# keonlee9420/Comprehensive-Transformer-TTS

Measured on AMD Instinct MI355X. Metric: mel-frames/sec (train step) LJSpeech batch=16, 1/2/4/8 MI355X, higher is better.
Workload: dtype f32; 1 GPU; LJSpeech transformer_fs2 batch=16/GPU seq<=128->mel<=1024x80; full train step fwd+loss+bwd+clip+Adam, dropout on; workload_detail=supervised durations (BASELINE configs[1]), global_batch=16, valid_frames_per_gpu=11992, padded_frames_per_gpu=16384, launch_mode=hipgraph(fwd+bwd | clip+adam), parallelism=dp1

## Files before the change

comprehensive-transformer-tts_amd/_lib.py:

```python
import ctypes as C
import os

_HERE = os.path.dirname(os.path.abspath(__file__))
LIB_PATH = os.environ.get("CTTS_LIB") or os.path.join(_HERE, "csrc", "libctts_hip.so")

_c_f32p = C.c_void_p
_i32, _i64, _f32, _u32, _vp = C.c_int32, C.c_int64, C.c_float, C.c_uint32, C.c_void_p


class GemmDesc(C.Structure):
    _fields_ = [
        ("A", _vp), ("B", _vp), ("C", _vp),
        ("M", _i32), ("N", _i32), ("K", _i32),
        ("lda", _i64), ("ldb", _i64), ("ldc", _i64),
        ("a_kc", _i32), ("b_kc", _i32),
        ("nb0", _i32), ("nb1", _i32),
        ("sA0", _i64), ("sA1", _i64), ("sB0", _i64), ("sB1", _i64), ("sC0", _i64), ("sC1", _i64),
        ("lens", _vp),
        ("lim_m", _i32), ("lim_n", _i32), ("lim_k", _i32),
        ("conv_T", _i32), ("conv_pad", _i32), ("conv_cin", _i32), ("conv_on_b", _i32),
        ("split_k", _i32),
        ("alpha", _f32),
        ("bias", _vp),
        ("Z", _vp), ("ldz", _i64),
# ... 83 lines not shown
    "ctts_gemm_takes_weight_stationary": [C.POINTER(GemmDesc)],
    "ctts_gemm_takes_bf16_split": [C.POINTER(GemmDesc)],
    "ctts_gemm_takes_planes": [C.POINTER(GemmDesc)],
    "ctts_split_planes": [C.POINTER(SplitTask), C.c_int, _vp],
    "ctts_rowdot_heads": [_vp, _vp, _vp, C.c_int, C.c_int, C.c_int, C.c_int, _vp],
    "ctts_mel_prepare": [_vp, C.c_int, C.c_int, _vp, _vp],
    "ctts_mel_spectrogram": [_vp, _vp, _vp, _vp, _vp, _vp, _vp, _i64, C.c_int, C.c_int, C.c_int, C.c_int, C.c_int, _f32, C.c_int, _vp, _vp],
    "ctts_mha_fwd": [_vp, _vp, _vp, _vp, C.c_int, C.c_int, C.c_int, C.c_int, _f32, _vp],
    "ctts_mha_bwd": [_vp, _vp, _vp, _vp, _vp, _vp, _vp, _vp, _vp, C.c_int, C.c_int, C.c_int, C.c_int, _f32, C.c_int, _vp, _vp],
    "ctts_relmha_fwd": [_vp, _vp, _vp, _vp, _vp, _vp, C.c_int, C.c_int, C.c_int, C.c_int, _f32, _f32, _vp, _u32, _vp],
    "ctts_relmha_bwd": [_vp, _vp, _vp, _vp, _vp, _vp, _vp, _vp, _vp, _vp, _vp, _vp, _vp, C.c_int, C.c_int, C.c_int, C.c_int,
                        _f32, _f32, _vp, _u32, _vp],
    "ctts_weighted_colsum": [_vp, _vp, _vp, _i64, C.c_int, _f32, C.c_int, _vp, _vp, _vp],
    "ctts_epilogue_bwd": [_vp, _vp, _vp, _vp, _vp, _vp, _i64, C.c_int, C.c_int, _f32, _vp, _u32, _f32, C.c_int, _vp, _vp, _vp],
    "ctts_row_tile_map": [_vp, C.c_int, C.c_int, C.c_int, _vp, _vp],
    "ctts_conv_weight_repack": [_vp, _vp, C.c_int, C.c_int, C.c_int, C.c_int, _vp],
    "ctts_lr_index": [_vp, C.c_int, C.c_int, _vp, C.c_int, C.c_int, C.c_int, _vp, _vp, _vp, _vp],
    "ctts_lr_gather_fwd": [_vp, _vp, _vp, C.c_int, C.c_int, C.c_int, C.c_int, _vp],
    "ctts_lr_gather_bwd": [_vp, _vp, _vp, C.c_int, C.c_int, C.c_int, C.c_int, _vp],
    "ctts_embedding_fwd": [_vp, _vp, _vp, _i64, C.c_int, C.c_int, _vp],
    "ctts_embedding_bwd": [_vp, _vp, _vp, _i64, C.c_int, C.c_int, C.c_int, C.c_int, _vp, _vp],
    "ctts_positions": [_vp, C.c_int, _i64, C.c_int, C.c_int, _vp, _vp],
    "ctts_cwt_pitch": [_vp, _i64, C.c_int, _vp, _vp, _f32, _vp, C.c_int, _f32, _f32, _f32, C.c_int, _vp, _vp, _vp, C.c_int, C.c_int, C.c_int, _vp],
    "ctts_layernorm_fwd": [_vp, _vp, _vp, _vp, _vp, _vp, C.c_int, C.c_int, _f32, _f32, _vp, _u32, _vp, _vp, _vp],
    "ctts_layernorm_bwd": [_vp, _vp, _vp, _vp, _vp, _vp, _vp, _vp, C.c_int, C.c_int, _f32, _vp, _u32, _vp, C.c_int, _vp, _vp, _vp, _vp],
    "ctts_colstats": [_vp, _vp, C.c_int, C.c_int, _vp, _vp],
    "ctts_bn_finalize": [_vp, C.c_int, C.c_int, _f32, _f32, _vp, _vp, _vp, _vp, _vp, _vp],
    "ctts_bn_apply": [_vp, _vp, _vp, _vp, _vp, _vp, C.c_int, C.c_int, C.c_int, _f32, _vp, _u32, _vp, _vp],
    "ctts_bn_bwd_reduce": [_vp, _vp, _vp, _vp, _vp, _vp, _vp, C.c_int, C.c_int, C.c_int, _f32, _vp, _u32, _vp, _vp],
    "ctts_bn_bwd_apply": [_vp, _vp, _vp, _vp, _vp, _vp, _vp, _vp, _vp, _vp, C.c_int, C.c_int, C.c_int, _f32, _vp,
# ... 76 lines not shown
    "ctts_stoi": [_vp, _vp, _vp, _vp, _vp, _vp, _vp, C.c_int, C.c_int, _vp, _vp],
    "ctts_si_sdr": [_vp, _vp, _vp, _vp, C.c_int, C.c_int, _vp, _vp],
    "ctts_mr_stft": [_vp, _vp, _vp, _vp, _vp, _vp, C.c_int, C.c_int, C.c_int, C.c_int, C.c_int, _vp, _vp],
    "ctts_comm_unique_id": [_vp],
    "ctts_comm_create": [C.POINTER(_vp), _i32, _i32, _vp],
    "ctts_comm_destroy": [_vp],
    "ctts_allreduce_mean": [_vp, _i64, _vp, _vp],
}
COMM_ID_BYTES = 128
EXPORTED_SYMBOLS = sorted(list(_SIGNATURES) + ["ctts_last_error", "ctts_version", "ctts_mha_supported", "ctts_relmha_workspace_floats",
                                               "ctts_mel_spectrogram_workspace_bytes", "ctts_gemm_workspace_bytes", "ctts_workspace_bytes",
                                               "ctts_workspace_error_word", "ctts_fastformer_workspace_floats",
                                               "ctts_griffinlim_workspace_bytes", "ctts_griffinlim_state_floats",
                                               "ctts_pitch_track_workspace_bytes", "ctts_trim_silence_workspace_bytes",
                                               "ctts_dtw_workspace_bytes", "ctts_loudness_workspace_bytes", "ctts_stoi_workspace_bytes",
                                               "ctts_si_sdr_workspace_bytes", "ctts_mr_stft_workspace_bytes"])
ADAM_STATE_FLOATS = 3 + 2048
ABI_VERSION = 2

_lib = None


class CttsError(RuntimeError):
    pass


def load():
    global _lib
    if _lib is not None:
        return _lib
    if not os.path.exists(LIB_PATH):
# ... 31 lines not shown
    lib.ctts_griffinlim_state_floats.argtypes = [C.c_int, C.c_int]
    lib.ctts_pitch_track_workspace_bytes.restype = C.c_size_t
    lib.ctts_pitch_track_workspace_bytes.argtypes = []
    lib.ctts_trim_silence_workspace_bytes.restype = C.c_size_t
    lib.ctts_trim_silence_workspace_bytes.argtypes = [C.c_int, C.c_int, C.c_int]
    lib.ctts_dtw_workspace_bytes.restype = C.c_size_t
    lib.ctts_dtw_workspace_bytes.argtypes = [C.c_int, C.c_int, C.c_int]
    lib.ctts_loudness_workspace_bytes.restype = C.c_size_t
    lib.ctts_loudness_workspace_bytes.argtypes = [C.c_int, C.c_int]
    lib.ctts_stoi_workspace_bytes.restype = C.c_size_t
    lib.ctts_stoi_workspace_bytes.argtypes = [C.c_int, C.c_int]
    lib.ctts_si_sdr_workspace_bytes.restype = C.c_size_t
    lib.ctts_si_sdr_workspace_bytes.argtypes = [C.c_int, C.c_int]
    lib.ctts_mr_stft_workspace_bytes.restype = C.c_size_t
    lib.ctts_mr_stft_workspace_bytes.argtypes = [C.c_int, C.c_int, C.c_int, C.c_int]
    lib.ctts_relmha_workspace_floats.restype = C.c_size_t
    lib.ctts_relmha_workspace_floats.argtypes = [C.c_int, C.c_int, C.c_int]
    _lib = lib
    return lib


def check(status, what):
    if status != 0:
        msg = load().ctts_last_error().decode(errors="replace")
        raise CttsError(f"{what} failed with status {status}: {msg}")
```

comprehensive-transformer-tts_amd/csrc/gemm.hip:

```cpp
#include "ctts_common.h"
#include "gemm_common.h"
#include <stdlib.h>
#include <type_traits>

namespace {

#ifndef CTTS_BK
#define CTTS_BK 32
#endif
#ifndef CTTS_GEMM_WAVES
#define CTTS_GEMM_WAVES 2
#endif
constexpr int BK = CTTS_BK;
constexpr int KC_LD = BK + 4;
constexpr int KCH = BK / 4;
static_assert(BK == 32 || BK == 64, "BK must be 32 or 64");


__device__ __forceinline__ bool rows_in_padding(const int32_t* row_lens, int row_T, int row_halo, int first, int last) {
  const int b0 = first / row_T;
  return b0 == last / row_T && (first - b0 * row_T) >= row_lens[b0] + row_halo;
}

__device__ __forceinline__ void batch_limits(const ctts_gemm_desc& d, int z0, bool apply, int& Mv, int& Nv, int& Kv) {
  Mv = d.M; Nv = d.N; Kv = d.K;
  if (apply && d.lens) {
    const int L = d.lens[z0];
    if (d.lim_m) Mv = min(Mv, L);
    if (d.lim_n) Nv = min(Nv, L);
    if (d.lim_k) Kv = min(Kv, L);
  }
}

__device__ __forceinline__ bool split_k_range(const ctts_gemm_desc& d, int Kv, int granule, int split, int& k_begin, int& k_end) {
  k_begin = 0; k_end = Kv;
  if (d.split_k > 1) {
    const GemmSplitRange s = gemm_split_range(Kv, d.split_k, granule, split);
    k_begin = s.k_begin; k_end = s.k_end;
    if (k_begin >= k_end) return false;
  }
  return true;
}

__device__ __forceinline__ void xcd_tile_order(int nwg, int tiles_n, bool scramble, int& wg, int& tm) {
  const int q8 = nwg >> 3, r8 = nwg & 7, xcd = blockIdx.x & 7, slot = blockIdx.x >> 3;
  wg = (xcd < r8 ? xcd * (q8 + 1) : r8 * (q8 + 1) + (xcd - r8) * q8) + slot;
// ... 363 lines not shown
  }
}

template <int BM, int BN, bool A_KC, bool B_KC, bool CONV, Fetch FETCH>
__global__ __launch_bounds__(256, CTTS_GEMM_WAVES) void gemm_tile_kernel(const ctts_gemm_desc d) {
  using FT = FetchTraits<FETCH>;
  constexpr int WAVES_N = BN >= 64 ? 2 : 1, WAVES_M = 4 / WAVES_N;
  constexpr int WM = BM / WAVES_M, WN = BN / WAVES_N, MT = WM / 32, NT = WN / 32;
  constexpr int A_LD = A_KC ? KC_LD : BM + 4;
  constexpr int B_LD = B_KC ? KC_LD : BN + 4;
  constexpr int A_SZ = A_KC ? BM * KC_LD : BK * (BM + 4);
  constexpr int B_SZ = B_KC ? BN * KC_LD : BK * (BN + 4);
  __shared__ __attribute__((aligned(16))) float smem[A_SZ + B_SZ];
  float* sA = smem;
  float* sB = smem + A_SZ;
  const int z = blockIdx.z;
  const int split = blockIdx.y;
  const int z0 = z / d.nb1, z1 = z - z0 * d.nb1;
  const bool limited = FT::kLensLimits && (FT::kLensGiven || d.lens);
  int Mv, Nv, Kv;
  batch_limits(d, z0, limited, Mv, Nv, Kv);
  const int tiles_n = (d.N + BN - 1) / BN;
  int wg, tm;
  bool scheduled_active = false;
  if (FT::kTileOrders && BM == 64 && A_KC && d.tile_map && !natural_order(d)) {
    wg = blockIdx.x;
    int r = wg / tiles_n;
    if (d.tile_group_n > 0) {
      const int g = d.tile_group_n, ngroups = tiles_n / g, mways = 8 / ngroups;
      const int x = blockIdx.x & 7, i = blockIdx.x >> 3;
      r = (i / g) * mways + x / ngroups;
      wg = r * tiles_n + (x % ngroups) * g + i % g;
    }
    tm = d.tile_map[1 + r];
    scheduled_active = FT::kTrustSchedule && r < d.tile_map[0];
  } else if (FT::kNaturalOrder || (FT::kTileOrders && natural_order(d))) {
    wg = blockIdx.x;
    tm = wg / tiles_n;
  } else {
    xcd_tile_order(gridDim.x, tiles_n, true, wg, tm);
  }
  const int row0 = tm * BM, col0 = (wg % tiles_n) * BN;
  float* Cb = d.C + z0 * d.sC0 + z1 * d.sC1;
  const bool zero_outside = limited && d.split_overwrite && d.split_k <= 1;
  if (row0 >= Mv || col0 >= Nv) {
    if (zero_outside && row0 < d.M && col0 < d.N) zero_outside_limits(d, Cb, row0, col0, BM, BN, Mv, Nv, true);
    return;
  }
  if (zero_outside && (row0 + BM > Mv || col0 + BN > Nv)) zero_outside_limits(d, Cb, row0, col0, BM, BN, Mv, Nv, false);
  float* Cs = Cb;
  if (d.split_k > 1) Cs += (long)split * d.M * d.ldc;
  if (A_KC && d.row_lens && !scheduled_active &&
      padded_tile_zeroed(d, FT::kPadFillOwnSplit ? Cs : Cb, row0, col0, BM, min(BN, Nv - col0), Mv)) return;
  int k_begin, k_end;
  if (!split_k_range(d, Kv, BK, split, k_begin, k_end)) return;

// ... 460 lines not shown
    const unsigned long long m = __ballot(a);
    if (a) map[1 + n_act + __popcll(m & ((1ULL << lane) - 1ULL))] = tm;
    n_act += __popcll(m);
  }
  int n_in = 0;
  for (int base = 0; base < tiles; base += 64) {
    const int tm = base + lane;
    const bool a = tm < tiles && inactive(tm);
    const unsigned long long m = __ballot(a);
    if (a) map[1 + n_act + n_in + __popcll(m & ((1ULL << lane) - 1ULL))] = tm;
    n_in += __popcll(m);
  }
  if (lane == 0) map[0] = n_act;
}

__global__ __launch_bounds__(256) void splitk_reduce_kernel(const ctts_gemm_desc d, int BM, int kround) {
  const int z = blockIdx.z, z0 = z / d.nb1, z1 = z - z0 * d.nb1;
  int Mv, Nv, Kv;
  batch_limits(d, z0, true, Mv, Nv, Kv);
  const bool ow = d.split_overwrite != 0;
  const int nact = Kv > 0 ? gemm_split_range(Kv, d.split_k, kround, 0).nonempty : 0;
  if (nact == 0 && !ow) return;
  const long ldp = gemm_partial_ld(d.N);
  const int n4 = (int)(ldp >> 2);
  const long e = (long)blockIdx.x * 256 + threadIdx.x;
  const int m = (int)(e / n4), n = (int)(e - (long)m * n4) * 4;
  if (m >= d.M || n >= d.N) return;
  bool live = m < Mv && n < Nv && nact > 0;
  if (live && d.a_kc && d.row_lens) {
    const int row0 = m / BM * BM;
// ... 30 lines not shown
int splitk_reduce(const ctts_gemm_desc& d, int BM, int kround, hipStream_t st) {
  const long e = (long)d.M * (gemm_partial_ld(d.N) / 4);
  hipLaunchKernelGGL(splitk_reduce_kernel, dim3((unsigned)((e + 255) / 256), 1, d.nb0 * d.nb1), dim3(256), 0, st, d, BM, kround);
  CTTS_CHECK_LAUNCH("ctts_gemm(split-K reduce)");
  return 0;
}
}

extern "C" int ctts_row_tile_map(const int32_t* row_lens, int row_T, int row_halo, int M, int32_t* tile_map, void* stream) {
  CTTS_REQUIRE(row_lens && tile_map && row_T > 0 && M >= 0, "ctts_row_tile_map: bad arguments");
  hipLaunchKernelGGL(row_tile_map_kernel, dim3(1), dim3(64), 0, (hipStream_t)stream, row_lens, row_T, row_halo, M, tile_map);
  CTTS_CHECK_LAUNCH("ctts_row_tile_map");
  return 0;
}

static bool x6_plan(const ctts_gemm_desc& d) {
  const int on = d.bf16_split;
  static const long min_tiles = ctts_env_int("CTTS_X6_MIN_TILES", 384);
  if (on < 1 || !d.a_kc || !d.b_kc || d.nb0 * d.nb1 != 1 || d.split_k > 1 || d.E || d.lens || d.conv_on_b) return false;
  if (d.K < 256 || d.K % BK || d.N % 128 || d.M < 1024) return false;
  if (d.conv_T > 0 && d.conv_cin % 4) return false;
  if (on != 2 && on != 4 && (long)((d.M + 127) / 128) * (d.N / 128) < min_tiles) return false;
  return vec_ok(d) && buf_ok(d);
}

static bool x6tn_plan(const ctts_gemm_desc& d) {
  static const int tn = ctts_env_int("CTTS_X6_TN", 1);
  static const long min_wg = ctts_env_int("CTTS_X6_TN_MIN_WG", 384);
  if (d.bf16_split < 1 || !tn || d.a_kc || d.b_kc || d.nb0 * d.nb1 != 1 || d.E || d.lens || d.epi_bwd) return false;
  if (d.M % 128 || d.N % 128 || d.K % BK || d.K < 2048) return false;
// ... 6 lines not shown
  const dim3 grid((d.M / 128) * (d.N / 128), d.split_k > 1 ? d.split_k : 1, 1);
  if (d.conv_T > 0) hipLaunchKernelGGL(gemm_x6tn_kernel<true>, grid, dim3(256), 0, st, d);
  else hipLaunchKernelGGL(gemm_x6tn_kernel<false>, grid, dim3(256), 0, st, d);
  CTTS_CHECK_LAUNCH("ctts_gemm(x6tn)");
  return 0;
}

static int x6_launch(const ctts_gemm_desc& d, hipStream_t st) {
  const int tiles = ((d.M + 127) / 128) * (d.N / 128);
  if (d.conv_T > 0) hipLaunchKernelGGL(gemm_x6_kernel<true>, dim3(tiles), dim3(256), 0, st, d);
  else hipLaunchKernelGGL(gemm_x6_kernel<false>, dim3(tiles), dim3(256), 0, st, d);
  CTTS_CHECK_LAUNCH("ctts_gemm(x6)");
  return 0;
}

struct GemmRoute {
  ctts_gemm_route_info info;
  bool split_fits;
  int tile_group_n;
  bool natural_order;
  union { PlArgs pl; PlwArgs plw; WsArgs ws; SkArgs sk; };
  GemmGrid grid;
};

static void tile_plan(const ctts_gemm_desc& d, bool x6tn, GemmRoute& r) {
  const long tiles128 = (long)((d.M + 127) / 128) * ((d.N + 127) / 128) * (d.split_k > 1 ? d.split_k : 1) * d.nb0 * d.nb1;
  static const int force_tile = ctts_env_int("CTTS_FORCE_TILE", 0);
  static const bool natural = getenv("CTTS_NATURAL_ORDER") != nullptr;
  static const int tile_group = ctts_env_int("CTTS_TILE_GROUP", -1);
  if (tile_group != 0 && d.tile_map && d.tile_map != reinterpret_cast<const int32_t*>(1)) {
    const int tn = (d.N + 63) / 64, tmn = (d.M + 63) / 64;
    const int g = tile_group > 0 ? tile_group : ((tn >= 8 && tn % 4 == 0) ? tn / 4 : 0);
    if (g > 0 && tn % g == 0) {
      const int ng = tn / g;
      if ((ng == 1 || ng == 2 || ng == 4 || ng == 8) && tmn % (8 / ng) == 0 && ((long)tmn * tn) % 8 == 0) r.tile_group_n = g;
    }
  }
  static const bool tn_natural = getenv("CTTS_TN_NATURAL") != nullptr;
  r.natural_order = (natural || (tn_natural && !d.a_kc && !d.b_kc)) && !d.tile_map;
  const bool aligned = vec_ok(d);
#ifdef CTTS_NO_BUF
  const bool buf_unaligned = false;
#else
  const bool buf_unaligned = !aligned && chunks_ok(d) && d.conv_T <= 0 && !(d.lens && (d.lim_m || d.lim_n || d.lim_k));
#endif
  r.info.tile_m = r.info.tile_n = 64;
  if (x6tn) { r.info.kind = CTTS_GEMM_X6TN; r.info.tile_m = r.info.tile_n = 128; }
  else if (!aligned && !(buf_unaligned && buf_ok(d))) r.info.kind = CTTS_GEMM_SCALAR64;
#ifndef CTTS_NO_BUF
  else if (buf_ok(d)) {
    static const int k2 = ctts_env_int("CTTS_K2_TILE", 640);
    static const int k2_mink = ctts_env_int("CTTS_K2_MIN_K", 256);
    static const int k2_tn = ctts_env_int("CTTS_K2_TN", 1);
    static const bool narrow = ctts_env_int("CTTS_NARROW_TILE", 1) != 0;
    if (force_tile == 128) { r.info.kind = CTTS_GEMM_BUF128; r.info.tile_m = r.info.tile_n = 128; }
    else if (k2 && (d.a_kc || (k2_tn && !d.b_kc)) && d.nb0 * d.nb1 == 1 && !d.lens && d.N >= 64 && d.M >= 256 && d.K >= k2_mink &&
             (long)((d.M + 63) / 64) * ((d.N + 63) / 64) * (d.split_k > 1 ? d.split_k : 1) <= k2) { r.info.kind = CTTS_GEMM_BUF_K2; r.info.tile_m = 32; }
    else if (narrow && d.N <= 32 && d.M >= 256 && d.conv_T <= 0 && !d.tile_map && !r.natural_order && !d.row_lens) { r.info.kind = CTTS_GEMM_BUF_NARROW; r.info.tile_m = 128; r.info.tile_n = 32; }
    else r.info.kind = CTTS_GEMM_BUF64;
  }
#endif
  else if (tiles128 >= 256 && d.N > 64 && (d.a_kc || d.b_kc)) { r.info.kind = CTTS_GEMM_VEC128; r.info.tile_m = r.info.tile_n = 128; }
  else r.info.kind = CTTS_GEMM_VEC64;
  r.info.k_granule = r.info.kind == CTTS_GEMM_BUF_K2 ? 2 * BK : BK;
}

static void gemm_route(const ctts_gemm_desc& d, GemmRoute& r, bool unbounded_room = false) {
  r.info = ctts_gemm_route_info{CTTS_GEMM_NONE, 128, 128, 1, 32};
  r.split_fits = true;
  r.tile_group_n = 0;
  r.natural_order = false;
  bool x6tn = false;
  if (ctts_gemm_pl_plan(d, r.pl, r.grid)) r.info.kind = CTTS_GEMM_PLANES;
// ... 15 lines not shown
static int gemm_validate(const ctts_gemm_desc* dp, ctts_gemm_desc& d) {
  CTTS_REQUIRE(dp != nullptr, "ctts_gemm: null descriptor");
  d = gemm_normalized(*dp);
  CTTS_REQUIRE(d.A && d.B && d.C, "ctts_gemm: null operand pointer");
  CTTS_REQUIRE(d.M >= 0 && d.N >= 0 && d.K >= 0, "ctts_gemm: negative dimension");
  if (d.M == 0 || d.N == 0) return 1;
  if (d.conv_T > 0) {
    CTTS_REQUIRE(d.conv_cin > 0 && (d.conv_cin % 4) == 0, "ctts_gemm: conv view needs cin %% 4 == 0 (got %d)", d.conv_cin);
    CTTS_REQUIRE(d.conv_on_b ? (!d.a_kc && !d.b_kc) : (d.a_kc != 0), "ctts_gemm: conv view on an unsupported operand layout");
  }
  CTTS_REQUIRE(d.p_drop >= 0.f && d.p_drop < 1.f, "ctts_gemm: p_drop out of range");
  CTTS_REQUIRE(!d.epi_bwd || (d.split_k <= 1 && !d.bias && !d.R && !d.rowscale && !d.E && (!d.act || d.Z)),
               "ctts_gemm: epi_bwd excludes bias, residual, rowscale, E and split-K, and needs Z when an activation is given");
  CTTS_REQUIRE(!d.E || (d.rowsub && d.split_k <= 1 && !d.bias && !d.act && d.p_drop == 0.f && !d.R && !d.rowscale && !d.Z),
               "ctts_gemm: the E/rowsub epilogue excludes bias, activation, dropout, residual, rowscale and split-K");
  return 0;
}

static int gemm_plan(const ctts_gemm_desc* dp, ctts_gemm_desc& d, GemmRoute& r) {
  const int rc = gemm_validate(dp, d);
  if (rc != 0) return rc;
  gemm_route(d, r);
  if (r.info.kind < CTTS_GEMM_X6TN || d.split_k <= 1) return 0;
  CTTS_REQUIRE(d.split_out || (d.sk_ws && d.sk_ws_bytes >= (int64_t)CTTS_WS_BYTES),
               "ctts_gemm: split_k > 1 needs the workspace (ctts_workspace_bytes() bytes, zero-filled once) in sk_ws - partial sums "
               "are added in a fixed order through it, the library has no floating-point atomics");
  CTTS_REQUIRE(r.split_fits, "ctts_gemm: split-K output [%d, %d] x %d batches does not fit the %s", d.M, d.N, d.nb0 * d.nb1,
               d.split_out ? "caller's split_out buffer" : "workspace");
  return 0;
}

extern "C" int ctts_gemm(const ctts_gemm_desc* dp, void* stream) {
  ctts_gemm_desc d;
  GemmRoute r;
  int rc = gemm_plan(dp, d, r);
  if (rc != 0) return rc < 0 ? rc : 0;
  hipStream_t st = reinterpret_cast<hipStream_t>(stream);
// ... 75 lines not shown
```

comprehensive-transformer-tts_amd/kernels.py:

```python
import collections
import ctypes as C

import torch

from . import _lib
from ._lib import GemmDesc

ACT_NONE, ACT_RELU, ACT_GELU, ACT_TANH, ACT_SWISH = 0, 1, 2, 3, 4


def _stream():
    return C.c_void_p(torch.cuda.current_stream().cuda_stream)


def _p(t, offset=0):
    if t is None:
        return None
    if not t.is_cuda:
        raise _lib.CttsError("ctts kernels need device (HIP) tensors; got a CPU tensor - no CPU fallback exists")
    return t.data_ptr() + offset * t.element_size()


def _f32c(t, name):
    if t.dtype != torch.float32 or not t.is_contiguous():
# ... 204 lines not shown
        d.conv_T, d.conv_pad, d.conv_cin = int(conv[0]), int(conv[1]), int(conv[2])
        d.conv_on_b = int(conv_on_b)
    d.split_k = int(split_k)
    d.alpha = float(alpha)
    d.bias = _p(bias)
    d.Z, d.ldz = _p(Z), int(ldz)
    d.act = int(act)
    d.p_drop = float(p_drop)
    d.seed = _p(seed)
    d.drop_offset = int(drop_offset)
    d.R, d.ldr = _p(R), int(ldr)
    d.rowscale = _p(rowscale)
    if row_lens is not None:
        d.row_lens, d.row_T, d.row_halo = _p(row_lens), int(row_T), int(row_halo)
        d.tile_map = _p(tile_map)
    d.E, d.rowsub = _p(E), _p(rowsub)
    d.epi_bwd = int(bool(epi_bwd))
    d.split_overwrite = int(bool(split_overwrite))
    if int(split_k) > 1 or a_planes is not None or ((SK_ENABLED if use_sk is None else use_sk) and nb0 * nb1 == 1 and M * N * K >= (1 << 24)):
        ws = gemm_workspace(A.device)
        d.sk_ws, d.sk_ws_bytes = ws.data_ptr(), ws.numel()
    return d


def gemm(A, B, Cout, M, N, K, lda, ldb, ldc, a_kc=True, b_kc=True, defer=False, **kw):
    d = _gemm_desc(A, B, Cout, M, N, K, lda, ldb, ldc, a_kc, b_kc, **kw)
    lib = _lib.load()
    if defer and _SINK is not None and d.split_k > 1 and d.nb0 * d.nb1 == 1 and ldc == N and N % 4 == 0:
        cnt, stride = C.c_int32(0), C.c_int64(0)
        if lib.ctts_gemm_split_plan(C.byref(d), C.byref(cnt), C.byref(stride)) == 1:
# ... 152 lines not shown
    return pl[:, :, q, :].reshape(pl.shape[0], -1)


def gemm_takes_weight_stationary(A, B, Cout, M, N, K, lda, ldb, ldc, a_kc=True, b_kc=True, **kw):
    return _gemm_takes("weight_stationary", (A, B, Cout, M, N, K, lda, ldb, ldc, a_kc, b_kc), kw)


def gemm_ws_enable(on):
    return bool(_lib.load().ctts_gemm_ws_enable(1 if on else 0))


def row_tile_map(row_lens, row_T, row_halo, M):
    tm = torch.empty(1 + (M + 63) // 64, dtype=torch.int32, device=row_lens.device)
    lib = _lib.load()
    _lib.check(lib.ctts_row_tile_map(_p(row_lens), int(row_T), int(row_halo), int(M), _p(tm), _stream()), "ctts_row_tile_map")
    return tm


def conv_dgrad_weights(weights):
    if not weights:
        return []
    outs = [torch.empty(cin, k * cout, dtype=torch.float32, device=w.device) for w, cout, cin, k in weights]
    arr = (_lib.RepackTask * len(weights))()
    for t, (w, cout, cin, k), o in zip(arr, weights, outs):
        t.src, t.dst, t.cout, t.cin, t.k = _p(_f32c(w, "conv weight (GEMM-major)")), _p(o), int(cout), int(cin), int(k)
    _lib.check(_lib.load().ctts_conv_dgrad_weights(arr, len(arr), _stream()), "ctts_conv_dgrad_weights")
    return outs


def conv_weight_repack(src, dst, cout, cin, k, mode):
# ... 1482 lines not shown
```

comprehensive-transformer-tts_amd/model.py:

```python
import json
import math
import os

import torch
import torch.nn as nn
import torch.nn.functional as F

from . import kernels as K
from . import ops
from .configs import N_SYMBOLS

F0_BIN = 256
F0_MEL_MIN = 1127 * math.log(1 + 50.0 / 700)
F0_MEL_MAX = 1127 * math.log(1 + 1100.0 / 700)


class _Linear(nn.Module):
    def __init__(self, cin, cout, bias=True):
        super().__init__()
        self.weight = nn.Parameter(torch.empty(cout, cin))
        self.bias = nn.Parameter(torch.empty(cout)) if bias else None


class _Conv(nn.Module):
# ... 124 lines not shown
        p = self.dropout if self.training else 0.0
        drop = self.drop_ctx if p > 0 else None
        nonpad, lens = mask_aux(pad_mask)
        if self.use_pos_embed:
            x = self.embed_positions.add_to(x.contiguous(), x, C, self.pos_embed_alpha, nonpad, p, drop)
        else:
            x = ops.rowscale_dropout(x, nonpad, 0.0, None)
        alpha = self.ksize ** -0.5
        pr = ops.PadRows(lens, T)
        for li, layer in enumerate(self.layers):
            op = layer.op
            if self._cut_prefix is not None:
                x = ops.stage_cut(x, f"{self._cut_prefix}.{li}")
            h, xr = ops.layer_norm_res(x, op.layer_norm1.weight, op.layer_norm1.bias, 1e-12)
            qkv = ops.linear(h, op.self_attn.in_proj_weight, pad_rows=pr)
            a = ops.self_attention(qkv, lens, self.num_heads)
            x = ops.linear(a, op.self_attn.out_proj.weight, None, residual=xr, rowscale=nonpad, p_drop=p, drop=drop, pad_rows=pr)
            h, xr = ops.layer_norm_res(x, op.layer_norm2.weight, op.layer_norm2.bias, 1e-12,
                                       planes_for=(op.ffn.conv1.weight.shape[0], self.ksize))
            link = ops.EpiLink()
            g = ops.conv1d(h, op.ffn.conv1.weight, op.ffn.conv1.bias, act=self.ffn_act, alpha=alpha, p_drop=p, drop=drop,
                           pad_rows=pr, link=link, link_role=1, padding=self.ffn_padding)
            x = ops.linear(g, op.ffn.ffn_2.weight, op.ffn.ffn_2.bias, residual=xr, rowscale=nonpad, p_drop=p, drop=drop,
                           pad_rows=pr, link=link, link_role=2)
        return ops.layer_norm(x, self.layer_norm.weight, self.layer_norm.bias, 1e-5, rowscale=nonpad)

    def forward(self, x, padding_mask=None):
        if padding_mask is None:
            padding_mask = x.abs().sum(-1).eq(0)
        return self.run(x, padding_mask), padding_mask

# ... 621 lines not shown
```

comprehensive-transformer-tts_amd/ops.py:

```python
import contextlib
import math
import os as _os

import torch

from . import kernels as K
from .kernels import ACT_NONE, ACT_RELU, ACT_GELU, ACT_TANH, ACT_SWISH


_FUSE_GRAD_ACCUM = False


def set_grad_accumulation_fusion(flag):
    global _FUSE_GRAD_ACCUM
    _FUSE_GRAD_ACCUM = bool(flag)


def grad_accumulation_fusion():
    return _FUSE_GRAD_ACCUM


def _grad_of(p):
    if not _FUSE_GRAD_ACCUM or p is None or not p.requires_grad:
        return None
# ... 447 lines not shown
    for (kind, w), pl in zip(slots, K.split_planes(mats)):
        _PLANES[kind][w.data_ptr()] = (pl, _wstamp(w))


def clear_dgrad_weights():
    _DGRAD_W.clear()
    _PLANES["fwd"].clear()
    _PLANES["dgrad"].clear()


class PadRows:

    def __init__(self, lens, T):
        self.lens, self.T = lens, int(T)
        self._maps = {}

    def tile_map(self, halo, M):
        key = (int(halo), int(M))
        if key not in self._maps:
            self._maps[key] = K.row_tile_map(self.lens, self.T, halo, M)
        return self._maps[key]


def _pad_rows(pad_rows):
    if pad_rows is None or isinstance(pad_rows, PadRows):
        return pad_rows
    return PadRows(pad_rows[0], pad_rows[1])


def linear(x, w, b=None, act=ACT_NONE, alpha=1.0, residual=None, rowscale=None, p_drop=0.0, drop=None, pad_rows=None, link=None,
           link_role=0):
    p_drop, seed, off = _drop_args(p_drop, drop)
    return _LinearConv.apply(x, w, b, residual, rowscale, act, alpha, p_drop, seed, off, 0, 0, _pad_rows(pad_rows), link, link_role)


def conv1d(x, w, b=None, act=ACT_NONE, alpha=1.0, residual=None, rowscale=None, p_drop=0.0, drop=None, pad_rows=None, link=None,
# ... 107 lines not shown
    Cc = x.shape[-1]
    return bool(x.is_cuda and K.PRODUCER_PLANES and K.plane_shape_ok(x.numel() // Cc, int(cout), int(ksize) * Cc, Cc))


def layer_norm_res(x, gamma, beta, eps, planes_for=None):
    want = planes_for is not None and consumer_takes_planes(x, *planes_for)
    return _LayerNormRes.apply(x, gamma, beta, eps, want)


def layer_norm(x, gamma, beta, eps, rowscale=None, p_drop=0.0, drop=None):
    p_drop, seed, off = _drop_args(p_drop, drop)
    return _LayerNorm.apply(x, gamma, beta, eps, rowscale, p_drop, seed, off)


_ATTN_SPLIT_K = int(_os.environ.get("CTTS_ATTN_SPLIT_K", "1"))


def _attn_split_k(nbatch, T, dh):
    tiles = -(-T // 64) * -(-dh // 64) * nbatch
    return _ATTN_SPLIT_K if (_ATTN_SPLIT_K > 1 and tiles < 1536 and T >= 512) else 1


_FUSED_ATTN = {"1": True, "0": False}.get(_os.environ.get("CTTS_FUSED_ATTN", "auto"), None)
_ATTN_Q_SPLIT = int(_os.environ.get("CTTS_ATTN_Q_SPLIT", "0"))


def set_fused_attention(flag):
    global _FUSED_ATTN
    _FUSED_ATTN = flag if flag is None else bool(flag)

# ... 15 lines not shown
        H = ctx.n_heads
        B, T, C3 = qkv.shape
        dh = C3 // 3 // H
        qs = _ATTN_Q_SPLIT if _ATTN_Q_SPLIT > 0 else (2 if (B * H * ((T + 31) // 32) <= 2048 and T >= 256) else 1)
        return K.mha_bwd(qkv, lens, out, dO.contiguous(), lse, H, dh ** -0.5, qs), None, None


def _heads(x, H, parts=1):
    B, T, Cc = x.shape
    return x.view(B, T, parts, H, Cc // (parts * H)).permute(2, 0, 3, 1, 4).unbind(0)


class _SelfAttention(torch.autograd.Function):

    @staticmethod
    def forward(ctx, qkv, lens, n_heads):
        qkv = qkv.contiguous()
        B, T, C3 = qkv.shape
        C = C3 // 3
        dh = C // n_heads
        q, k, v = _heads(qkv, n_heads, 3)
        S = torch.empty(B, n_heads, T, T, dtype=torch.float32, device=qkv.device)
        K.bgemm(q, k.transpose(-1, -2), S, lens=lens, lim=(1, 1, 0), alpha=dh ** -0.5)
        K.softmax_fwd(S, lens, B, n_heads, T)
        sk = _attn_split_k(B * n_heads, T, dh)
        out = torch.empty(B, T, C, dtype=torch.float32, device=qkv.device)
        K.bgemm(S, v, _heads(out, n_heads)[0], lens=lens, lim=(1, 0, 1), split_k=sk, split_overwrite=True)
        ctx.save_for_backward(qkv, S, lens, out)
        ctx.n_heads = n_heads
        return out

    @staticmethod
    def backward(ctx, dO):
        qkv, P, lens, O = ctx.saved_tensors
        H = ctx.n_heads
        dO = dO.contiguous()
        B, T, C3 = qkv.shape
        dh = C3 // 3 // H
        scale = dh ** -0.5
        sk = _attn_split_k(B * H, T, dh)
        dqkv = torch.empty_like(qkv)
        (q, k, v), (dq, dk, dv), (dOh,) = _heads(qkv, H, 3), _heads(dqkv, H, 3), _heads(dO, H)
        K.bgemm(P.transpose(-1, -2), dOh, dv, lens=lens, lim=(1, 0, 1), split_k=sk, split_overwrite=True)
        Dv = K.rowdot_heads(dO, O, H)
        dP = torch.empty_like(P)
        K.bgemm(dOh, v.transpose(-1, -2), dP, lens=lens, lim=(1, 1, 0), E=P, rowsub=Dv)
        K.bgemm(dP, k, dq, lens=lens, lim=(1, 0, 1), alpha=scale, split_k=sk, split_overwrite=True)
        K.bgemm(dP.transpose(-1, -2), q, dk, lens=lens, lim=(1, 0, 1), alpha=scale, split_k=sk, split_overwrite=True)
        return dqkv, None, None


def self_attention(qkv, lens_i32, n_heads):
    want = _FUSED_ATTN if _FUSED_ATTN is not None else not (torch.is_grad_enabled() and qkv.requires_grad)
    if want and K.mha_supported(qkv.shape[-1] // 3, n_heads):
        return _FusedSelfAttention.apply(qkv, lens_i32, n_heads)
    return _SelfAttention.apply(qkv, lens_i32, n_heads)


class _LRGather(torch.autograd.Function):
    @staticmethod
    def forward(ctx, x, mel2ph, cum):
        x = x.contiguous()
        ctx.save_for_backward(cum)
        ctx.Ts = x.shape[1]
        return K.lr_gather_fwd(x, mel2ph)

    @staticmethod
    def backward(ctx, dy):
        (cum,) = ctx.saved_tensors
        return K.lr_gather_bwd(dy.contiguous(), cum, ctx.Ts), None, None

# ... 819 lines not shown
```

include/ctts.h:

```cpp
#ifndef CTTS_H
#define CTTS_H
#include <stddef.h>
#include <stdint.h>

#ifdef __cplusplus
extern "C" {
#endif

const char* ctts_last_error(void);
int ctts_version(void);

typedef struct ctts_gemm_desc {
  const float* A; const float* B; float* C;
  int32_t M, N, K;
  int64_t lda, ldb, ldc;
  int32_t a_kc, b_kc;
  int32_t nb0, nb1;
  int64_t sA0, sA1, sB0, sB1, sC0, sC1;
  const int32_t* lens;
  int32_t lim_m, lim_n, lim_k;
  int32_t conv_T, conv_pad, conv_cin, conv_on_b;
  int32_t split_k;
  float alpha;
  const float* bias;
// ... 49 lines not shown
int ctts_gemm_takes_planes(const ctts_gemm_desc* d);
typedef struct ctts_split_task { const float* src; uint16_t* dst; int64_t rows, cols, ld; } ctts_split_task;
int ctts_split_planes(const ctts_split_task* tasks, int ntasks, void* stream);

int ctts_rowdot_heads(const float* a, const float* b, float* out, int B, int T, int H, int dh, void* stream);

int ctts_weighted_colsum(const float* x, const float* w, float* out, int64_t rows, int C, float scale, int accumulate, void* ws, float* parts,
                         void* stream);

int ctts_epilogue_bwd(const float* dy, const float* rowscale, const float* z, float* dz, float* gm, float* dbias, int64_t rows, int C,
                      int act, float p_drop, const uint64_t* seed, uint32_t drop_offset, float bias_scale, int accumulate_bias,
                      void* ws, float* parts, void* stream);

int ctts_row_tile_map(const int32_t* row_lens, int row_T, int row_halo, int M, int32_t* tile_map, void* stream);

int ctts_conv_weight_repack(const float* src, float* dst, int cout, int cin, int k, int mode, void* stream);

int ctts_lr_index(const void* dur, int dur_is_float, int round_mode, const uint8_t* pad, int B, int Ts, int Tm,
                  int32_t* mel2ph, int64_t* mel_len, int32_t* cum, void* stream);
int ctts_lr_gather_fwd(const float* x, const int32_t* mel2ph, float* out, int B, int Ts, int Tm, int C, void* stream);
int ctts_lr_gather_bwd(const float* dy, const int32_t* cum, float* dx, int B, int Ts, int Tm, int C, void* stream);

int ctts_cwt_pitch(const float* spec, int64_t ld_spec, int nscale, const float* f0_mean, const float* f0_std, float std_scale,
                   const float* uv, int uv_chan, float eps, float mel_min, float mel_max, int f0_bin, float* f0, float* f0_denorm,
                   int64_t* ids, int B, int T, int width, void* stream);

int ctts_positions(const void* src, int src_is_float, int64_t stride, int B, int T, int32_t* pos, void* stream);

int ctts_layernorm_fwd(const float* x, const float* gamma, const float* beta, float* y, float* mean, float* rstd,
                       int rows, int C, float eps, float p_drop, const uint64_t* seed, uint32_t drop_offset,
// ... 246 lines not shown
```

Before: 681,300 mel-frames/s.

## Schedule batched attention GEMM tiles by per-batch work with a device-built plan

Adds a device-side batch tile plan for variable-length batched GEMMs in the unfused self-attention path. It lists the active tiles of every batch, orders them by K-work in a snake pattern across CU bins, and lets the 64x64 buffer kernel launch only the active tiles, returning early for the rest. The goal is to cut idle workgroups and load imbalance from padded sequences in the attention bgemms. In exchange it adds an extra plan kernel per shape, a per-workgroup indirection through the plan, and new routing constraints (no split-K, buf64 kernel only).

```diff
diff --git a/comprehensive-transformer-tts_amd/_lib.py b/comprehensive-transformer-tts_amd/_lib.py
--- a/comprehensive-transformer-tts_amd/_lib.py
+++ b/comprehensive-transformer-tts_amd/_lib.py
@@ -121,6 +121,7 @@
     "ctts_weighted_colsum": [_vp, _vp, _vp, _i64, C.c_int, _f32, C.c_int, _vp, _vp, _vp],
     "ctts_epilogue_bwd": [_vp, _vp, _vp, _vp, _vp, _vp, _i64, C.c_int, C.c_int, _f32, _vp, _u32, _f32, C.c_int, _vp, _vp, _vp],
     "ctts_row_tile_map": [_vp, C.c_int, C.c_int, C.c_int, _vp, _vp],
+    "ctts_batch_tile_map": [_vp] + [C.c_int] * 9 + [_vp, C.c_size_t, _vp],
     "ctts_conv_weight_repack": [_vp, _vp, C.c_int, C.c_int, C.c_int, C.c_int, _vp],
     "ctts_lr_index": [_vp, C.c_int, C.c_int, _vp, C.c_int, C.c_int, C.c_int, _vp, _vp, _vp, _vp],
     "ctts_lr_gather_fwd": [_vp, _vp, _vp, C.c_int, C.c_int, C.c_int, C.c_int, _vp],
@@ -227,7 +228,8 @@
                                                "ctts_griffinlim_workspace_bytes", "ctts_griffinlim_state_floats",
                                                "ctts_pitch_track_workspace_bytes", "ctts_trim_silence_workspace_bytes",
                                                "ctts_dtw_workspace_bytes", "ctts_loudness_workspace_bytes", "ctts_stoi_workspace_bytes",
-                                               "ctts_si_sdr_workspace_bytes", "ctts_mr_stft_workspace_bytes"])
+                                               "ctts_si_sdr_workspace_bytes", "ctts_mr_stft_workspace_bytes",
+                                               "ctts_batch_tile_map_ints"])
 ADAM_STATE_FLOATS = 3 + 2048
 ABI_VERSION = 2
 
@@ -289,6 +291,8 @@
     lib.ctts_si_sdr_workspace_bytes.argtypes = [C.c_int, C.c_int]
     lib.ctts_mr_stft_workspace_bytes.restype = C.c_size_t
     lib.ctts_mr_stft_workspace_bytes.argtypes = [C.c_int, C.c_int, C.c_int, C.c_int]
+    lib.ctts_batch_tile_map_ints.restype = C.c_size_t
+    lib.ctts_batch_tile_map_ints.argtypes = [C.c_int, C.c_int, C.c_int, C.c_int]
     lib.ctts_relmha_workspace_floats.restype = C.c_size_t
     lib.ctts_relmha_workspace_floats.argtypes = [C.c_int, C.c_int, C.c_int]
     _lib = lib
diff --git a/comprehensive-transformer-tts_amd/csrc/batch_plan.h b/comprehensive-transformer-tts_amd/csrc/batch_plan.h
--- /dev/null
+++ b/comprehensive-transformer-tts_amd/csrc/batch_plan.h
@@ -0,0 +1,76 @@
+#pragma once
+#include <stdint.h>
+#ifdef __HIPCC__
+#define BP_HD __host__ __device__ __forceinline__
+#else
+#define BP_HD inline
+#endif
+
+struct BatchPlanGeom {
+  int M, N, K;
+  int BM, BN, BK;
+  int nbatch, nb1;
+  int lim_m, lim_n, lim_k;
+  int write_all;
+  int nbins;
+};
+
+constexpr int BATCH_PLAN_HDR = 4;
+
+BP_HD int batch_plan_tiles_m(const BatchPlanGeom& g) { return (g.M + g.BM - 1) / g.BM; }
+BP_HD int batch_plan_tiles_n(const BatchPlanGeom& g) { return (g.N + g.BN - 1) / g.BN; }
+BP_HD long batch_plan_items(const BatchPlanGeom& g) { return (long)g.nbatch * batch_plan_tiles_m(g) * batch_plan_tiles_n(g); }
+
+BP_HD bool batch_plan_fits(const BatchPlanGeom& g) {
+  const long tiles = (long)batch_plan_tiles_m(g) * batch_plan_tiles_n(g);
+  return g.nbatch >= 1 && g.nb1 >= 1 && g.nbins >= 1 && tiles >= 1 && tiles <= 65536 && g.nbatch <= 32767 &&
+         tiles * g.nbatch * g.nbatch <= (1L << 26);
+}
+BP_HD int32_t batch_plan_pack(int z, int tile) { return (int32_t)((z << 16) | tile); }
+BP_HD void batch_plan_unpack(int32_t e, int& z, int& tile) { z = (int)((uint32_t)e >> 16); tile = e & 0xFFFF; }
+
+BP_HD int32_t batch_plan_key(const BatchPlanGeom& g) {
+  return (int32_t)((g.lim_m & 1) | (g.lim_n & 1) << 1 | (g.lim_k & 1) << 2 | (g.write_all & 1) << 3 | (batch_plan_tiles_n(g) & 0xFFF) << 4 |
+                   (g.BM & 0xFF) << 16 | (g.BN & 0xFF) << 24);
+}
+
+struct BatchPlanBatch {
+  int work;
+  int act_m, act_n;
+};
+
+BP_HD BatchPlanBatch batch_plan_batch(const BatchPlanGeom& g, int L) {
+  const int Mv = g.lim_m && L < g.M ? L : g.M, Nv = g.lim_n && L < g.N ? L : g.N, Kv = g.lim_k && L < g.K ? L : g.K;
+  BatchPlanBatch b;
+  b.work = Kv > 0 ? (Kv + g.BK - 1) / g.BK : 0;
+  b.act_m = Mv > 0 ? (Mv + g.BM - 1) / g.BM : 0;
+  b.act_n = Nv > 0 ? (Nv + g.BN - 1) / g.BN : 0;
+  if (b.act_m == 0 || b.act_n == 0) b.act_m = b.act_n = 0;
+  return b;
+}
+
+BP_HD int batch_plan_snake(int p, int n_active, int nbins) {
+  const int layer = p / nbins, r = p - layer * nbins;
+  const int width = n_active - layer * nbins < nbins ? n_active - layer * nbins : nbins;
+  return layer * nbins + ((layer & 1) ? width - 1 - r : r);
+}
+
+BP_HD int batch_plan_slot(const BatchPlanGeom& g, const int32_t* lens, int z, int tile, int& n_active) {
+  const int tiles_n = batch_plan_tiles_n(g), tiles = batch_plan_tiles_m(g) * tiles_n;
+  const BatchPlanBatch me = batch_plan_batch(g, lens[z / g.nb1]);
+  int act_before = 0, rest_before = 0, total = 0;
+  for (int y = 0; y < g.nbatch; ++y) {
+    const BatchPlanBatch o = batch_plan_batch(g, lens[y / g.nb1]);
+    const int a = o.act_m * o.act_n;
+    total += a;
+    if (o.work > me.work || (o.work == me.work && y < z)) act_before += a;
+    if (y < z) rest_before += tiles - a;
+  }
+  n_active = total;
+  const int tm = tile / tiles_n, tn = tile - tm * tiles_n;
+  const int act_in = (tm < me.act_m ? tm : me.act_m) * me.act_n + (tm < me.act_m ? (tn < me.act_n ? tn : me.act_n) : 0);
+  if (tm < me.act_m && tn < me.act_n) return batch_plan_snake(act_before + act_in, total, g.nbins);
+  return total + rest_before + (tile - act_in);
+}
+
+BP_HD int batch_plan_listed(const BatchPlanGeom& g, int n_active) { return g.write_all ? (int)batch_plan_items(g) : n_active; }
diff --git a/comprehensive-transformer-tts_amd/csrc/gemm.hip b/comprehensive-transformer-tts_amd/csrc/gemm.hip
--- a/comprehensive-transformer-tts_amd/csrc/gemm.hip
+++ b/comprehensive-transformer-tts_amd/csrc/gemm.hip
@@ -1,5 +1,6 @@
 #include "ctts_common.h"
 #include "gemm_common.h"
+#include "batch_plan.h"
 #include <stdlib.h>
 #include <type_traits>
 
@@ -30,6 +31,11 @@
     if (d.lim_n) Nv = min(Nv, L);
     if (d.lim_k) Kv = min(Kv, L);
   }
+}
+
+__host__ __device__ __forceinline__ BatchPlanGeom batch_plan_geom(const ctts_gemm_desc& d, int BM, int BN, int nbins) {
+  return BatchPlanGeom{d.M, d.N, d.K, BM, BN, BK, d.nb0 * d.nb1, d.nb1, d.lim_m != 0, d.lim_n != 0, d.lim_k != 0,
+                       d.split_overwrite != 0 && d.split_k <= 1, nbins};
 }
 
 __device__ __forceinline__ bool split_k_range(const ctts_gemm_desc& d, int Kv, int granule, int split, int& k_begin, int& k_end) {
@@ -423,16 +429,25 @@
   __shared__ __attribute__((aligned(16))) float smem[A_SZ + B_SZ];
   float* sA = smem;
   float* sB = smem + A_SZ;
-  const int z = blockIdx.z;
+  int z = blockIdx.z;
   const int split = blockIdx.y;
-  const int z0 = z / d.nb1, z1 = z - z0 * d.nb1;
   const bool limited = FT::kLensLimits && (FT::kLensGiven || d.lens);
-  int Mv, Nv, Kv;
-  batch_limits(d, z0, limited, Mv, Nv, Kv);
   const int tiles_n = (d.N + BN - 1) / BN;
   int wg, tm;
   bool scheduled_active = false;
-  if (FT::kTileOrders && BM == 64 && A_KC && d.tile_map && !natural_order(d)) {
+  if constexpr (FT::kNaturalOrder) {
+    wg = blockIdx.x;
+    if (d.tile_map && !natural_order(d)) {
+      const int32_t* plan = d.tile_map;
+      const unsigned lin = blockIdx.z * gridDim.x + blockIdx.x;
+      if (plan[2] == (int32_t)(gridDim.x * gridDim.z) && plan[3] == batch_plan_key(batch_plan_geom(d, BM, BN, 1))) {
+        if (lin >= (unsigned)plan[1]) return;
+        batch_plan_unpack(plan[BATCH_PLAN_HDR + lin], z, wg);
+        if (z >= (int)gridDim.z || wg >= (int)gridDim.x) return;
+      }
+    }
+    tm = wg / tiles_n;
+  } else if (FT::kTileOrders && BM == 64 && A_KC && d.tile_map && !natural_order(d)) {
     wg = blockIdx.x;
     int r = wg / tiles_n;
     if (d.tile_group_n > 0) {
@@ -443,12 +458,15 @@
     }
     tm = d.tile_map[1 + r];
     scheduled_active = FT::kTrustSchedule && r < d.tile_map[0];
-  } else if (FT::kNaturalOrder || (FT::kTileOrders && natural_order(d))) {
+  } else if (FT::kTileOrders && natural_order(d)) {
     wg = blockIdx.x;
     tm = wg / tiles_n;
   } else {
     xcd_tile_order(gridDim.x, tiles_n, true, wg, tm);
   }
+  const int z0 = z / d.nb1, z1 = z - z0 * d.nb1;
+  int Mv, Nv, Kv;
+  batch_limits(d, z0, limited, Mv, Nv, Kv);
   const int row0 = tm * BM, col0 = (wg % tiles_n) * BN;
   float* Cb = d.C + z0 * d.sC0 + z1 * d.sC1;
   const bool zero_outside = limited && d.split_overwrite && d.split_k <= 1;
@@ -939,6 +957,22 @@
   if (lane == 0) map[0] = n_act;
 }
 
+__global__ __launch_bounds__(256) void batch_tile_map_kernel(const BatchPlanGeom g, const int32_t* __restrict__ lens, int32_t* __restrict__ map) {
+  const int n_items = (int)batch_plan_items(g), tiles = n_items / g.nbatch;
+  for (int i = blockIdx.x * 256 + threadIdx.x; i < n_items; i += gridDim.x * 256) {
+    const int z = i / tiles, tile = i - z * tiles;
+    int n_active;
+    const int slot = batch_plan_slot(g, lens, z, tile, n_active);
+    map[BATCH_PLAN_HDR + slot] = batch_plan_pack(z, tile);
+    if (i == 0) {
+      map[0] = n_active;
+      map[1] = batch_plan_listed(g, n_active);
+      map[2] = n_items;
+      map[3] = batch_plan_key(g);
+    }
+  }
+}
+
 __global__ __launch_bounds__(256) void splitk_reduce_kernel(const ctts_gemm_desc d, int BM, int kround) {
   const int z = blockIdx.z, z0 = z / d.nb1, z1 = z - z0 * d.nb1;
   int Mv, Nv, Kv;
@@ -999,6 +1033,38 @@
   return 0;
 }
 
+static BatchPlanGeom batch_map_geom(int nb0, int nb1, int M, int N, int K, int lim_m, int lim_n, int lim_k, int write_all) {
+  static int cus = 0;
+  if (!cus) {
+    int dev = 0;
+    hipDeviceProp_t prop;
+    cus = (hipGetDevice(&dev) == hipSuccess && hipGetDeviceProperties(&prop, dev) == hipSuccess && prop.multiProcessorCount > 0)
+              ? prop.multiProcessorCount : 256;
+    cus = ctts_env_int("CTTS_BATCH_BINS", cus);
+    if (cus < 1) cus = 256;
+  }
+  return BatchPlanGeom{M, N, K, 64, 64, BK, nb0 * nb1, nb1, lim_m != 0, lim_n != 0, lim_k != 0, write_all != 0, cus};
+}
+
+extern "C" size_t ctts_batch_tile_map_ints(int nb0, int nb1, int M, int N) {
+  if (nb0 < 1 || nb1 < 1 || M < 1 || N < 1 || (long)nb0 * nb1 > 32767) return 0;
+  const BatchPlanGeom g = batch_map_geom(nb0, nb1, M, N, 1, 0, 0, 0, 0);
+  return batch_plan_fits(g) ? (size_t)(BATCH_PLAN_HDR + batch_plan_items(g)) : 0;
+}
+
+extern "C" int ctts_batch_tile_map(const int32_t* lens, int nb0, int nb1, int M, int N, int K, int lim_m, int lim_n, int lim_k,
+                                   int write_all, int32_t* tile_map, size_t map_ints, void* stream) {
+  CTTS_REQUIRE(lens && tile_map && K >= 0, "ctts_batch_tile_map: bad arguments");
+  const size_t need = ctts_batch_tile_map_ints(nb0, nb1, M, N);
+  CTTS_REQUIRE(need > 0, "ctts_batch_tile_map: %d x %d batches of [%d, %d] do not fit a plan (ctts_batch_tile_map_ints)", nb0, nb1, M, N);
+  CTTS_REQUIRE(map_ints >= need, "ctts_batch_tile_map: tile_map holds %zu int32, %zu needed", map_ints, need);
+  const BatchPlanGeom g = batch_map_geom(nb0, nb1, M, N, K, lim_m, lim_n, lim_k, write_all);
+  const long blocks = (batch_plan_items(g) + 255) / 256;
+  hipLaunchKernelGGL(batch_tile_map_kernel, dim3((unsigned)(blocks < 64 ? blocks : 64)), dim3(256), 0, (hipStream_t)stream, g, lens, tile_map);
+  CTTS_CHECK_LAUNCH("ctts_batch_tile_map");
+  return 0;
+}
+
 static bool x6_plan(const ctts_gemm_desc& d) {
   const int on = d.bf16_split;
   static const long min_tiles = ctts_env_int("CTTS_X6_MIN_TILES", 384);
@@ -1035,6 +1101,10 @@
   return 0;
 }
 
+static bool batch_plan_given(const ctts_gemm_desc& d) {
+  return d.tile_map && d.tile_map != reinterpret_cast<const int32_t*>(1) && d.lens && (d.lim_m || d.lim_n || d.lim_k);
+}
+
 struct GemmRoute {
   ctts_gemm_route_info info;
   bool split_fits;
@@ -1049,7 +1119,7 @@
   static const int force_tile = ctts_env_int("CTTS_FORCE_TILE", 0);
   static const bool natural = getenv("CTTS_NATURAL_ORDER") != nullptr;
   static const int tile_group = ctts_env_int("CTTS_TILE_GROUP", -1);
-  if (tile_group != 0 && d.tile_map && d.tile_map != reinterpret_cast<const int32_t*>(1)) {
+  if (tile_group != 0 && d.tile_map && d.tile_map != reinterpret_cast<const int32_t*>(1) && !batch_plan_given(d)) {
     const int tn = (d.N + 63) / 64, tmn = (d.M + 63) / 64;
     const int g = tile_group > 0 ? tile_group : ((tn >= 8 && tn % 4 == 0) ? tn / 4 : 0);
     if (g > 0 && tn % g == 0) {
@@ -1077,7 +1147,7 @@
     if (force_tile == 128) { r.info.kind = CTTS_GEMM_BUF128; r.info.tile_m = r.info.tile_n = 128; }
     else if (k2 && (d.a_kc || (k2_tn && !d.b_kc)) && d.nb0 * d.nb1 == 1 && !d.lens && d.N >= 64 && d.M >= 256 && d.K >= k2_mink &&
              (long)((d.M + 63) / 64) * ((d.N + 63) / 64) * (d.split_k > 1 ? d.split_k : 1) <= k2) { r.info.kind = CTTS_GEMM_BUF_K2; r.info.tile_m = 32; }
-    else if (narrow && d.N <= 32 && d.M >= 256 && d.conv_T <= 0 && !d.tile_map && !r.natural_order && !d.row_lens) { r.info.kind = CTTS_GEMM_BUF_NARROW; r.info.tile_m = 128; r.info.tile_n = 32; }
+    else if (narrow && d.N <= 32 && d.M >= 256 && d.conv_T <= 0 && (!d.tile_map || batch_plan_given(d)) && !r.natural_order && !d.row_lens) { r.info.kind = CTTS_GEMM_BUF_NARROW; r.info.tile_m = 128; r.info.tile_n = 32; }
     else r.info.kind = CTTS_GEMM_BUF64;
   }
 #endif
@@ -1123,6 +1193,9 @@
                "ctts_gemm: epi_bwd excludes bias, residual, rowscale, E and split-K, and needs Z when an activation is given");
   CTTS_REQUIRE(!d.E || (d.rowsub && d.split_k <= 1 && !d.bias && !d.act && d.p_drop == 0.f && !d.R && !d.rowscale && !d.Z),
                "ctts_gemm: the E/rowsub epilogue excludes bias, activation, dropout, residual, rowscale and split-K");
+  CTTS_REQUIRE(!batch_plan_given(d) || (!d.row_lens && d.split_k <= 1 && batch_plan_fits(batch_plan_geom(d, 64, 64, 1))),
+               "ctts_gemm: a batch tile plan (tile_map on a launch with length limits) excludes row_lens and split-K, and the batches "
+               "must fit one (ctts_batch_tile_map_ints)");
   return 0;
 }
 
@@ -1130,6 +1203,8 @@
   const int rc = gemm_validate(dp, d);
   if (rc != 0) return rc;
   gemm_route(d, r);
+  CTTS_REQUIRE(!batch_plan_given(d) || r.info.kind == CTTS_GEMM_BUF64,
+               "ctts_gemm: a batch tile plan was given, but the launch does not run on the 64 x 64 buffer kernel (route kind %d)", r.info.kind);
   if (r.info.kind < CTTS_GEMM_X6TN || d.split_k <= 1) return 0;
   CTTS_REQUIRE(d.split_out || (d.sk_ws && d.sk_ws_bytes >= (int64_t)CTTS_WS_BYTES),
                "ctts_gemm: split_k > 1 needs the workspace (ctts_workspace_bytes() bytes, zero-filled once) in sk_ws - partial sums "
diff --git a/comprehensive-transformer-tts_amd/kernels.py b/comprehensive-transformer-tts_amd/kernels.py
--- a/comprehensive-transformer-tts_amd/kernels.py
+++ b/comprehensive-transformer-tts_amd/kernels.py
@@ -242,6 +242,8 @@
     if row_lens is not None:
         d.row_lens, d.row_T, d.row_halo = _p(row_lens), int(row_T), int(row_halo)
         d.tile_map = _p(tile_map)
+    elif lens is not None:
+        d.tile_map = _p(tile_map)
     d.E, d.rowsub = _p(E), _p(rowsub)
     d.epi_bwd = int(bool(epi_bwd))
     d.split_overwrite = int(bool(split_overwrite))
@@ -424,6 +426,17 @@
     tm = torch.empty(1 + (M + 63) // 64, dtype=torch.int32, device=row_lens.device)
     lib = _lib.load()
     _lib.check(lib.ctts_row_tile_map(_p(row_lens), int(row_T), int(row_halo), int(M), _p(tm), _stream()), "ctts_row_tile_map")
+    return tm
+
+
+def batch_tile_map(lens, nb1, M, N, K, lim, write_all):
+    lib = _lib.load()
+    n = lib.ctts_batch_tile_map_ints(int(lens.numel()), int(nb1), int(M), int(N))
+    if n == 0:
+        return None
+    tm = torch.empty(n, dtype=torch.int32, device=lens.device)
+    _lib.check(lib.ctts_batch_tile_map(_p(lens), int(lens.numel()), int(nb1), int(M), int(N), int(K), int(lim[0]), int(lim[1]), int(lim[2]),
+                                       int(bool(write_all)), _p(tm), n, _stream()), "ctts_batch_tile_map")
     return tm
 
 
diff --git a/comprehensive-transformer-tts_amd/model.py b/comprehensive-transformer-tts_amd/model.py
--- a/comprehensive-transformer-tts_amd/model.py
+++ b/comprehensive-transformer-tts_amd/model.py
@@ -162,7 +162,7 @@
                 x = ops.stage_cut(x, f"{self._cut_prefix}.{li}")
             h, xr = ops.layer_norm_res(x, op.layer_norm1.weight, op.layer_norm1.bias, 1e-12)
             qkv = ops.linear(h, op.self_attn.in_proj_weight, pad_rows=pr)
-            a = ops.self_attention(qkv, lens, self.num_heads)
+            a = ops.self_attention(qkv, lens, self.num_heads, pad_rows=pr)
             x = ops.linear(a, op.self_attn.out_proj.weight, None, residual=xr, rowscale=nonpad, p_drop=p, drop=drop, pad_rows=pr)
             h, xr = ops.layer_norm_res(x, op.layer_norm2.weight, op.layer_norm2.bias, 1e-12,
                                        planes_for=(op.ffn.conv1.weight.shape[0], self.ksize))
diff --git a/comprehensive-transformer-tts_amd/ops.py b/comprehensive-transformer-tts_amd/ops.py
--- a/comprehensive-transformer-tts_amd/ops.py
+++ b/comprehensive-transformer-tts_amd/ops.py
@@ -485,12 +485,27 @@
     def __init__(self, lens, T):
         self.lens, self.T = lens, int(T)
         self._maps = {}
+        self._batch_maps = {}
 
     def tile_map(self, halo, M):
         key = (int(halo), int(M))
         if key not in self._maps:
             self._maps[key] = K.row_tile_map(self.lens, self.T, halo, M)
         return self._maps[key]
+
+
+    def batch_map(self, A, B, Cout, lim, write_all):
+        key = (tuple(Cout.shape), int(A.shape[-1]), tuple(lim), bool(write_all))
+        if key not in self._batch_maps:
+            plan = None
+            nb1, (M, N), Kd = (Cout.shape[1] if Cout.dim() == 4 else 1), Cout.shape[-2:], A.shape[-1]
+            if Cout.is_cuda and Cout.dim() >= 3 and Cout.shape[0] * nb1 * -(-M // 64) * -(-N // 64) > _BATCH_ORDER_MIN_ITEMS:
+                args, views = K.gemm_views(A, B, Cout, lens=self.lens)
+                route = K.gemm_route(*args, **views, lens=self.lens, lim=lim, split_overwrite=write_all)
+                if route.kind == "buf64":
+                    plan = K.batch_tile_map(self.lens, nb1, M, N, Kd, lim, write_all)
+            self._batch_maps[key] = plan
+        return self._batch_maps[key]
 
 
 def _pad_rows(pad_rows):
@@ -628,6 +643,8 @@
 
 
 _ATTN_SPLIT_K = int(_os.environ.get("CTTS_ATTN_SPLIT_K", "1"))
+_BATCH_ORDER = _os.environ.get("CTTS_BATCH_ORDER", "balanced")
+_BATCH_ORDER_MIN_ITEMS = 256
 
 
 def _attn_split_k(nbatch, T, dh):
@@ -673,26 +690,33 @@
 class _SelfAttention(torch.autograd.Function):
 
     @staticmethod
-    def forward(ctx, qkv, lens, n_heads):
+    def _bgemm(pr, A, B, Cout, lens, lim, split_k=1, split_overwrite=False, **kw):
+        plan = pr.batch_map(A, B, Cout, lim, split_overwrite) if (pr is not None and split_k <= 1) else None
+        return K.bgemm(A, B, Cout, lens=lens, lim=lim, split_k=split_k, split_overwrite=split_overwrite, tile_map=plan, **kw)
+
+    @staticmethod
+    def forward(ctx, qkv, lens, n_heads, pad_rows=None):
         qkv = qkv.contiguous()
         B, T, C3 = qkv.shape
         C = C3 // 3
         dh = C // n_heads
+        pr = None if _BATCH_ORDER == "natural" else (pad_rows if pad_rows is not None else PadRows(lens, T))
         q, k, v = _heads(qkv, n_heads, 3)
         S = torch.empty(B, n_heads, T, T, dtype=torch.float32, device=qkv.device)
-        K.bgemm(q, k.transpose(-1, -2), S, lens=lens, lim=(1, 1, 0), alpha=dh ** -0.5)
+        _SelfAttention._bgemm(pr, q, k.transpose(-1, -2), S, lens, (1, 1, 0), alpha=dh ** -0.5)
         K.softmax_fwd(S, lens, B, n_heads, T)
         sk = _attn_split_k(B * n_heads, T, dh)
         out = torch.empty(B, T, C, dtype=torch.float32, device=qkv.device)
-        K.bgemm(S, v, _heads(out, n_heads)[0], lens=lens, lim=(1, 0, 1), split_k=sk, split_overwrite=True)
+        _SelfAttention._bgemm(pr, S, v, _heads(out, n_heads)[0], lens, (1, 0, 1), split_k=sk, split_overwrite=True)
         ctx.save_for_backward(qkv, S, lens, out)
         ctx.n_heads = n_heads
+        ctx.pad_rows = pr
         return out
 
     @staticmethod
     def backward(ctx, dO):
         qkv, P, lens, O = ctx.saved_tensors
-        H = ctx.n_heads
+        H, pr, bg = ctx.n_heads, ctx.pad_rows, _SelfAttention._bgemm
         dO = dO.contiguous()
         B, T, C3 = qkv.shape
         dh = C3 // 3 // H
@@ -700,20 +724,20 @@
         sk = _attn_split_k(B * H, T, dh)
         dqkv = torch.empty_like(qkv)
         (q, k, v), (dq, dk, dv), (dOh,) = _heads(qkv, H, 3), _heads(dqkv, H, 3), _heads(dO, H)
-        K.bgemm(P.transpose(-1, -2), dOh, dv, lens=lens, lim=(1, 0, 1), split_k=sk, split_overwrite=True)
+        bg(pr, P.transpose(-1, -2), dOh, dv, lens, (1, 0, 1), split_k=sk, split_overwrite=True)
         Dv = K.rowdot_heads(dO, O, H)
         dP = torch.empty_like(P)
-        K.bgemm(dOh, v.transpose(-1, -2), dP, lens=lens, lim=(1, 1, 0), E=P, rowsub=Dv)
-        K.bgemm(dP, k, dq, lens=lens, lim=(1, 0, 1), alpha=scale, split_k=sk, split_overwrite=True)
-        K.bgemm(dP.transpose(-1, -2), q, dk, lens=lens, lim=(1, 0, 1), alpha=scale, split_k=sk, split_overwrite=True)
-        return dqkv, None, None
-
-
-def self_attention(qkv, lens_i32, n_heads):
+        bg(pr, dOh, v.transpose(-1, -2), dP, lens, (1, 1, 0), E=P, rowsub=Dv)
+        bg(pr, dP, k, dq, lens, (1, 0, 1), alpha=scale, split_k=sk, split_overwrite=True)
+        bg(pr, dP.transpose(-1, -2), q, dk, lens, (1, 0, 1), alpha=scale, split_k=sk, split_overwrite=True)
+        return dqkv, None, None, None
+
+
+def self_attention(qkv, lens_i32, n_heads, pad_rows=None):
     want = _FUSED_ATTN if _FUSED_ATTN is not None else not (torch.is_grad_enabled() and qkv.requires_grad)
     if want and K.mha_supported(qkv.shape[-1] // 3, n_heads):
         return _FusedSelfAttention.apply(qkv, lens_i32, n_heads)
-    return _SelfAttention.apply(qkv, lens_i32, n_heads)
+    return _SelfAttention.apply(qkv, lens_i32, n_heads, pad_rows)
 
 
 class _LRGather(torch.autograd.Function):
diff --git a/include/ctts.h b/include/ctts.h
--- a/include/ctts.h
+++ b/include/ctts.h
@@ -87,6 +87,10 @@
 
 int ctts_row_tile_map(const int32_t* row_lens, int row_T, int row_halo, int M, int32_t* tile_map, void* stream);
 
+size_t ctts_batch_tile_map_ints(int nb0, int nb1, int M, int N);
+int ctts_batch_tile_map(const int32_t* lens, int nb0, int nb1, int M, int N, int K, int lim_m, int lim_n, int lim_k, int write_all,
+                        int32_t* tile_map, size_t map_ints, void* stream);
+
 int ctts_conv_weight_repack(const float* src, float* dst, int cout, int cin, int k, int mode, void* stream);
 
 int ctts_lr_index(const void* dur, int dur_is_float, int round_mode, const uint8_t* pad, int B, int Ts, int Tm,
```

Result: faster. 691,200 mel-frames/s (median of 6 runs) (+1.5%).
